# gwall-ceres/HighRes-net

Hardware: AMD Instinct MI355X
Metric: SR frames/sec (384x384 out) at B=32, n_views=32 (higher is better)
Workload: dtype bf16

## Files before the change

highres-net_amd/hrnet_hip/csrc/conv3x3.h:

```cpp
#pragma once
#include "common.h"

#define CONV_TILE_H 8
#define CONV_TILE_W 32
#define CONV_STEP_BYTES 8192

struct ConvParams {
    const void* in;
    const void* stack;
    int in_pair;
    void* out;
    const void* res;
    const float* alphas;
    const void* wpk;
    const float* bias;
    const float* slope;
    int M, H, W;
    int pair_h, pair_last, pair_vs;
    int out_h, out_vs;
    int res_mode;
    int alpha_vs, res_vs;
    int relu;
    const float* scale;
    size_t in_lo, stack_lo, out_lo, res_lo;
    const float* only_if_nonpos;
};

static inline size_t conv_packed_elems(int cin, int cout) { return (size_t)cin * cout * 9; }

int hrn_launch_conv3x3(int dt, int cin, int cout, const ConvParams& p, hipStream_t stream, bool general_only);

int hrn_launch_conv3x3_r64(const ConvParams& p, hipStream_t stream);

int hrn_launch_conv3x3_v6(int cin, int cout, const ConvParams& p, hipStream_t stream);

int hrn_launch_conv3x3_v6x3(int cin, int cout, const ConvParams& p, hipStream_t stream);

int hrn_launch_conv_pack(int dt, int cin, int cout, const float* w_oihw, void* packed, hipStream_t stream);
```

highres-net_amd/hrnet_hip/csrc/conv3x3_r64.hip:

```cpp
#include <type_traits>
#include "conv3x3.h"

namespace {

constexpr int HALO_H = CONV_TILE_H + 2;
constexpr int HALO_W = CONV_TILE_W + 2;
constexpr int IN_BYTES = HALO_H * HALO_W * 128;
constexpr int W_BYTES = 9 * 64 * 128;
constexpr int LDS_BYTES = W_BYTES + 2 * IN_BYTES + 256;

__device__ __forceinline__ void lds_done_then_barrier() {
    asm volatile("s_waitcnt lgkmcnt(0)" ::: "memory");
    __builtin_amdgcn_s_barrier();
    asm volatile("" ::: "memory");
}

__device__ __forceinline__ float raw_max(float a, float b) {
    float y;
    asm("v_max_f32 %0, %1, %2" : "=v"(y) : "v"(a), "v"(b));
    return y;
}

__device__ __attribute__((aligned(16))) unsigned hrn_r64_zero16[4];

template <bool RES>
__global__ __launch_bounds__(512, 2) void conv3x3_r64_kernel(const ConvParams p) {
    if (p.only_if_nonpos && p.only_if_nonpos[0] > 0.f) return;
    extern __shared__ __attribute__((aligned(16))) unsigned char smem[];
    unsigned char* w_lds = smem;
    float* bias_lds = (float*)(smem + W_BYTES + 2 * IN_BYTES);

    const int tid = threadIdx.x;
    const int lane = tid & 63;
    const int wave = __builtin_amdgcn_readfirstlane(tid >> 6);
    const int team = wave >> 2, tw = wave & 3;
    unsigned char* in_lds = smem + W_BYTES + team * IN_BYTES;
    const int r = lane & 31, hh = lane >> 5;
    const int H = p.H, W = p.W;
    const size_t hw = (size_t)H * W;
    const unsigned tiles_x = (W + CONV_TILE_W - 1) / CONV_TILE_W;
    const unsigned tiles_y = (H + CONV_TILE_H - 1) / CONV_TILE_H;
    const unsigned tiles = tiles_x * tiles_y;
    const unsigned total = tiles * (unsigned)p.M;
    const unsigned G = gridDim.x;
    const unsigned bid = blockIdx.x;
    const unsigned slot = (G & 7) == 0 ? (bid & 7) * (G >> 3) + (bid >> 3) : bid;
    if (slot >= total) return;
    const int ntl = (int)((total - slot + G - 1) / G);
    const int nmine = (ntl + 1 - team) >> 1;

    unsigned cur_m = (slot + team * G) / tiles, cur_t = (slot + team * G) - cur_m * tiles;
    const unsigned step_m = (2 * G) / tiles, step_t = 2 * G - step_m * tiles;

    {
        const u32x4* wg = (const u32x4*)p.wpk;
#pragma unroll
        for (int j = 0; j < W_BYTES / 16 / 512; ++j) {
            const int idx = tid + j * 512;
            const int row = idx >> 3, c = idx & 7;
            *(u32x4*)(w_lds + row * 128 + ((c ^ ((row >> 1) & 7)) << 4)) = wg[idx];
        }
        if (tid < 64) bias_lds[tid] = p.bias[tid];
    }

    unsigned voff[11], cm_lo = 0, cm_hi = 0;
    if (!RES) {
#pragma unroll
        for (int jj = 0; jj < 11; ++jj) {
            const int j = tw + 4 * jj;
            const int pix = j * 8 + (lane >> 3);
            const int py = pix / HALO_W, px = pix - py * HALO_W;
            voff[jj] = (unsigned)((py * W + px) * 128 + (((lane & 7) ^ ((pix >> 1) & 7)) << 4));
            unsigned cls = (py == 0 ? 1u : 0u) | (py == HALO_H - 1 ? 2u : 0u) | (px == 0 ? 4u : 0u) | (px == HALO_W - 1 ? 8u : 0u);
            if (pix >= HALO_H * HALO_W) cls = 0;
            if (jj < 8) cm_lo |= cls << (4 * jj); else cm_hi |= cls << (4 * (jj - 8));
        }
    }
    unsigned pend_F = 0;
    auto issue = [&](unsigned m, unsigned t) __attribute__((always_inline)) {
        const int ty = t / tiles_x;
        const int y0 = ty * CONV_TILE_H, x0 = (t - ty * tiles_x) * CONV_TILE_W;
        const unsigned char* base = (const unsigned char*)p.in + (size_t)m * hw * 128;
        const bool fast = !RES && y0 + CONV_TILE_H <= H && x0 + CONV_TILE_W <= W && (m > 0 || y0 > 0) &&
                          ((int)m + 1 < p.M || (size_t)(y0 + CONV_TILE_H) * W + x0 + CONV_TILE_W < hw);
        pend_F = 0;
        if (fast) {
            const unsigned char* hb = base + ((long)(y0 - 1) * W + (x0 - 1)) * 128;
#pragma unroll
            for (int jj = 0; jj < 11; ++jj) {
                const int j = tw + 4 * jj;
                if (j < 43) {
                    if (jj < 10 || j * 8 + (lane >> 3) < HALO_H * HALO_W)
                        __builtin_amdgcn_global_load_lds((const __attribute__((address_space(1))) void*)(hb + voff[jj]),
                                                         (__attribute__((address_space(3))) void*)(in_lds + j * 1024), 16, 0, 0);
                }
            }
            pend_F = (y0 == 0 ? 1u : 0u) | (y0 + CONV_TILE_H == H ? 2u : 0u) | (x0 == 0 ? 4u : 0u) | (x0 + CONV_TILE_W == W ? 8u : 0u);
            __builtin_amdgcn_sched_barrier(0);
            return;
        }
        int lq = lane;
        asm volatile("" : "+v"(lq));
#pragma unroll
        for (int jj = 0; jj < 11; ++jj) {
            const int j = tw + 4 * jj;
            if (j < 43) {
                const int pix = j * 8 + (lq >> 3);
                const int lc = (lq & 7) ^ ((pix >> 1) & 7);
                const int py = pix / HALO_W, px = pix - py * HALO_W;
                const int gy = y0 - 1 + py, gx = x0 - 1 + px;
                const bool ok = (unsigned)gy < (unsigned)H && (unsigned)gx < (unsigned)W;
                const unsigned char* src = ok ? base + (unsigned)((gy * W + gx) * 128 + lc * 16) : (const unsigned char*)hrn_r64_zero16;
                if (pix < HALO_H * HALO_W)
                    __builtin_amdgcn_global_load_lds((const __attribute__((address_space(1))) void*)src,
                                                     (__attribute__((address_space(3))) void*)(in_lds + j * 1024), 16, 0, 0);
            }
        }
        __builtin_amdgcn_sched_barrier(0);
    };
    auto fix_borders = [&]() __attribute__((always_inline)) {
        if (!RES && pend_F) {
            const unsigned fm = pend_F * 0x11111111u;
            const unsigned hit_lo = cm_lo & fm, hit_hi = cm_hi & fm;
            const u32x4 z = {0u, 0u, 0u, 0u};
#pragma unroll
            for (int jj = 0; jj < 11; ++jj) {
                const int j = tw + 4 * jj;
                if (j < 43) {
                    const unsigned h = jj < 8 ? (hit_lo >> (4 * jj)) & 15u : (hit_hi >> (4 * (jj - 8))) & 15u;
                    if (h) *(u32x4*)(in_lds + j * 1024 + lane * 16) = z;
                }
            }
        }
    };

    const bool has_slope = p.slope != nullptr;
    const float slope = has_slope ? p.slope[0] : 0.f;
    const bool slope01 = slope >= 0.f && slope <= 1.f;
    const unsigned lds0 = (unsigned)(__UINTPTR_TYPE__)(__attribute__((address_space(3))) unsigned char*)smem;
    unsigned a_off[4], a_off_hi[4], b_off[4][3];
#pragma unroll
    for (int ks = 0; ks < 4; ++ks) {
        a_off[ks] = lds0 + r * 128 + (((ks * 2 + hh) ^ ((r >> 1) & 7)) << 4);
        a_off_hi[ks] = a_off[ks] + 4 * 8192;
    }
#pragma unroll
    for (int row = 0; row < 4; ++row)
#pragma unroll
        for (int kx = 0; kx < 3; ++kx) {
            const int pix = (2 * tw + row) * HALO_W + r + kx;
            b_off[row][kx] = lds0 + (unsigned)(W_BYTES + team * IN_BYTES) + (((unsigned)pix << 7) | ((unsigned)(((pix >> 1) & 7) ^ hh) << 4));
        }

    f32x16 acc[2][2];

    auto multiply = [&]() __attribute__((always_inline)) {
#pragma unroll
        for (int cb = 0; cb < 2; ++cb)
#pragma unroll
            for (int g = 0; g < 4; ++g) {
                const f32x4 b = *(const f32x4*)(bias_lds + cb * 32 + 8 * g + 4 * hh);
#pragma unroll
                for (int j = 0; j < 4; ++j) { acc[cb][0][4 * g + j] = b[j]; acc[cb][1][4 * g + j] = b[j]; }
            }
        constexpr int NK = 36;
        bf16x8 fa[3][2], fb[3][2];
        auto rd = [&](bf16x8& dst, unsigned addr, int imm) __attribute__((always_inline)) {
            asm volatile("ds_read_b128 %0, %1 offset:%2" : "=v"(dst) : "v"(addr), "n"(imm));
        };
        auto load_part = [&](int i, int part) __attribute__((always_inline)) {
            const int s_ = i % 3, tap = i >> 2, ks = i & 3;
            const int ky = tap / 3, kx = tap - ky * 3;
            if (part < 2) {
                rd(fa[s_][part], tap < 4 ? a_off[ks] : a_off_hi[ks], (tap < 4 ? tap : tap - 4) * 8192 + part * 4096);
            } else {
                unsigned kbits = 0;
                if (ks) asm volatile("s_mov_b32 %0, %1" : "=s"(kbits) : "n"(ks << 5));
                rd(fb[s_][part - 2], b_off[part - 2 + ky][kx] ^ kbits, 0);
            }
        };
        asm volatile("s_waitcnt lgkmcnt(0)" ::: "memory");
        __builtin_amdgcn_s_setprio(3);
#pragma unroll
        for (int i = 0; i < 2; ++i)
#pragma unroll
            for (int part = 0; part < 4; ++part) load_part(i, part);
        __builtin_amdgcn_sched_barrier(0);
#pragma unroll
        for (int i = 0; i < NK; ++i) {
            const int s_ = i % 3;
            const bool more = i + 2 < NK;
            if (i < NK - 1) asm volatile("s_waitcnt lgkmcnt(5)" : "+v"(fa[s_][0]), "+v"(fb[s_][0]));
            else asm volatile("s_waitcnt lgkmcnt(1)" : "+v"(fa[s_][0]), "+v"(fb[s_][0]));
            acc[0][0] = __builtin_amdgcn_mfma_f32_32x32x16_bf16(fa[s_][0], fb[s_][0], acc[0][0], 0, 0, 0);
            if (more) load_part(i + 2, 0);
            __builtin_amdgcn_sched_barrier(0);
            if (more) asm volatile("s_waitcnt lgkmcnt(5)" : "+v"(fb[s_][1]));
            else if (i == NK - 2) asm volatile("s_waitcnt lgkmcnt(4)" : "+v"(fb[s_][1]));
            else asm volatile("s_waitcnt lgkmcnt(0)" : "+v"(fb[s_][1]));
            acc[0][1] = __builtin_amdgcn_mfma_f32_32x32x16_bf16(fa[s_][0], fb[s_][1], acc[0][1], 0, 0, 0);
            if (more) load_part(i + 2, 1);
            __builtin_amdgcn_sched_barrier(0);
            asm volatile("" : "+v"(fa[s_][1]));
            acc[1][0] = __builtin_amdgcn_mfma_f32_32x32x16_bf16(fa[s_][1], fb[s_][0], acc[1][0], 0, 0, 0);
            if (more) load_part(i + 2, 2);
            __builtin_amdgcn_sched_barrier(0);
            acc[1][1] = __builtin_amdgcn_mfma_f32_32x32x16_bf16(fa[s_][1], fb[s_][1], acc[1][1], 0, 0, 0);
            if (more) load_part(i + 2, 3);
            __builtin_amdgcn_sched_barrier(0);
        }
        __builtin_amdgcn_s_setprio(0);
    };

    u32x4 resv[2][4];
    float res_alpha = 1.f;
    auto fetch_residual = [&]() __attribute__((always_inline)) {
        const int m = (int)cur_m;
        const int ty = cur_t / tiles_x;
        const int y0 = ty * CONV_TILE_H, x0 = (cur_t - ty * tiles_x) * CONV_TILE_W;
        const unsigned char* rbase = (const unsigned char*)p.res + (size_t)m * hw * 128;
        if (p.res_mode == 3) {
            const int ob = m / p.out_h, oi = m - ob * p.out_h;
            rbase = (const unsigned char*)p.res + ((size_t)ob * p.res_vs + oi) * hw * 128;
            res_alpha = p.alphas ? p.alphas[(size_t)ob * p.alpha_vs + (p.pair_last - oi)] : 1.f;
        }
#pragma unroll
        for (int pb = 0; pb < 2; ++pb) {
            const int gy = y0 + 2 * tw + pb, gyc = gy < H ? gy : H - 1;
#pragma unroll
            for (int j = 0; j < 4; ++j) {
                const int gxj = x0 + (r & ~3) + j, gxjc = gxj < W ? gxj : W - 1;
                resv[pb][j] = __builtin_nontemporal_load((const u32x4*)(rbase + (unsigned)((gyc * W + gxjc) * 128 + hh * 64 + (r & 3) * 16)));
            }
        }
    };

    auto finish = [&](bool more) __attribute__((always_inline)) {
        const int m = (int)cur_m;
        const int ty = cur_t / tiles_x;
        const int y0 = ty * CONV_TILE_H, x0 = (cur_t - ty * tiles_x) * CONV_TILE_W;
        cur_t += step_t; cur_m += step_m;
        if (cur_t >= tiles) { cur_t -= tiles; ++cur_m; }
        size_t oimg = (size_t)m;
        int ob = 0, oi = 0;
        if (p.out_h > 0) { ob = m / p.out_h; oi = m - ob * p.out_h; oimg = (size_t)ob * p.out_vs + oi; }
        unsigned char* outp = (unsigned char*)p.out + (oimg * hw + (size_t)y0 * W + x0) * 128;
        if (RES) {
#pragma unroll
            for (int pb = 0; pb < 2; ++pb)
#pragma unroll
                for (int g = 0; g < 4; ++g) asm volatile("" :: "v"(resv[pb][g]));
            asm volatile("" :: "v"(res_alpha));
        }
        if (more) issue(cur_m, cur_t);
        auto epilogue = [&](auto act_c) __attribute__((always_inline)) {
        constexpr int ACT = decltype(act_c)::value;
#pragma unroll
        for (int pb = 0; pb < 2; ++pb) {
            const int gy = y0 + 2 * tw + pb;
            u32x4 uu[4];
            if (RES) quad_transpose(resv[pb], (lane & 1) != 0, (lane & 2) != 0);
#pragma unroll
            for (int g = 0; g < 4; ++g) {
                float xa[4], xb[4];
#pragma unroll
                for (int j = 0; j < 4; ++j) { xa[j] = acc[0][pb][4 * g + j]; xb[j] = acc[1][pb][4 * g + j]; }
                if (ACT == 1) {
#pragma unroll
                    for (int j = 0; j < 4; ++j) { xa[j] = raw_max(xa[j], slope * xa[j]); xb[j] = raw_max(xb[j], slope * xb[j]); }
                } else if (ACT == 2) {
#pragma unroll
                    for (int j = 0; j < 4; ++j) { xa[j] = xa[j] >= 0.f ? xa[j] : slope * xa[j]; xb[j] = xb[j] >= 0.f ? xb[j] : slope * xb[j]; }
                }
                u32x4 u;
                if (RES) {
                    float v[8];
#pragma unroll
                    for (int j = 0; j < 4; ++j) {
                        const u32x2 sw = __builtin_amdgcn_permlane32_swap(__float_as_uint(xa[j]), __float_as_uint(xb[j]), false, false);
                        v[j] = __uint_as_float(sw[0]);
                        v[4 + j] = __uint_as_float(sw[1]);
                    }
                    const u32x4 rq = resv[pb][g];
#pragma unroll
                    for (int j = 0; j < 4; ++j) {
                        const float r0 = __uint_as_float(rq[j] << 16), r1 = __uint_as_float(rq[j] & 0xffff0000u);
                        if (p.res_mode == 3) { v[2 * j] = r0 + res_alpha * v[2 * j]; v[2 * j + 1] = r1 + res_alpha * v[2 * j + 1]; }
                        else { v[2 * j] += r0; v[2 * j + 1] += r1; }
                    }
#pragma unroll
                    for (int j = 0; j < 4; ++j) u[j] = pack2_bf16(v[2 * j], v[2 * j + 1]);
                } else {
                    const u32x2 s0 = __builtin_amdgcn_permlane32_swap(pack2_bf16(xa[0], xa[1]), pack2_bf16(xb[0], xb[1]), false, false);
                    const u32x2 s1 = __builtin_amdgcn_permlane32_swap(pack2_bf16(xa[2], xa[3]), pack2_bf16(xb[2], xb[3]), false, false);
                    u[0] = s0[0]; u[1] = s1[0]; u[2] = s0[1]; u[3] = s1[1];
                }
                uu[g] = u;
            }
            {
                quad_transpose(uu, (lane & 1) != 0, (lane & 2) != 0);
                unsigned char* oq = outp + (unsigned)(((2 * tw + pb) * W + (r & ~3)) * 128 + hh * 64 + (r & 3) * 16);
#pragma unroll
                for (int j = 0; j < 4; ++j)
                    if (gy < H && x0 + (r & ~3) + j < W) __builtin_nontemporal_store(uu[j], (u32x4*)(oq + j * 128));
            }
        }
        };
        if (!has_slope) epilogue(std::integral_constant<int, 0>{});
        else if (slope01) epilogue(std::integral_constant<int, 1>{});
        else epilogue(std::integral_constant<int, 2>{});
        {
            const int nst = 4 * ((y0 + 2 * tw < H) + (y0 + 2 * tw + 1 < H));
            if (nst == 8) asm volatile("s_waitcnt vmcnt(8)" ::: "memory");
            else if (nst == 4) asm volatile("s_waitcnt vmcnt(4)" ::: "memory");
            else asm volatile("s_waitcnt vmcnt(0)" ::: "memory");
        }
        fix_borders();
    };

    if (nmine > 0) issue(cur_m, cur_t);
    asm volatile("s_waitcnt vmcnt(0)" ::: "memory");
    fix_borders();
    lds_done_then_barrier();

    for (int ph = 0; ph <= ntl; ++ph) {
        const int q = ph - team;
        if (q >= 0) {
            const int k = q >> 1;
            if (k < nmine) {
                if ((q & 1) == 0) { if (RES) fetch_residual(); multiply(); }
                else finish(k + 1 < nmine);
            }
        }
        if (ph < ntl) lds_done_then_barrier();
    }
}


template <bool RES>
int launch_r64(const ConvParams& p, long grid, hipStream_t stream) {
    { const int rc_lds = hrn_allow_lds((const void*)conv3x3_r64_kernel<RES>, LDS_BYTES); if (rc_lds) return rc_lds; }
    hipLaunchKernelGGL(conv3x3_r64_kernel<RES>, dim3((unsigned)grid), dim3(512), LDS_BYTES, stream, p);
    HRN_LAUNCH_CHECK();
    return 0;
}

}

int hrn_launch_conv3x3_r64(const ConvParams& p, hipStream_t stream) {
    if (p.scale || p.relu || p.in_pair || p.res_mode == 2) return -100;
    static_assert(LDS_BYTES <= 160 * 1024, "LDS budget");
    const long tiles = (long)((p.W + CONV_TILE_W - 1) / CONV_TILE_W) * ((p.H + CONV_TILE_H - 1) / CONV_TILE_H);
    const long total = tiles * p.M;
    HRN_CHECK(total > 0, -2, "conv3x3_r64: bad tile count %ld", total);
    if (total >= (1L << 30) || (long)p.H * p.W * 128 >= (1L << 31)) return -100;
    long grid = hrn_device_cus();
    if (total < grid) grid = total;
    if (grid >= 8) grid &= ~7L;
    const double px = (double)p.M * p.H * p.W;
    HrnProfScope prof(p.res_mode ? "conv3x3_bf16_64x64+res" : "conv3x3_bf16_64x64", 2.0 * 64 * 64 * 9 * px,
                      px * 2 * (64 + 64 + (p.res_mode ? 64 : 0)), stream);
    return p.res_mode ? launch_r64<true>(p, grid, stream) : launch_r64<false>(p, grid, stream);
}
```

Measured before the change: 1969.

## Walk conv tiles in vertical strips with a ring buffer reusing halo rows

The 64x64 3x3 conv kernel now assigns each team a vertical segment of consecutive tiles in one column, rather than scattered tiles. The input LDS tile becomes a ring buffer, so the two halo rows shared with the previous tile are kept and only the new rows are loaded. This cuts redundant global loads of halo rows by roughly 20 percent of input traffic. A host heuristic picks the segment length to balance the load across CUs. The cost is more complex indexing, per-tile recomputation of the B-operand offsets, and possible load imbalance or tail effects.

```diff
diff --git a/highres-net_amd/hrnet_hip/csrc/conv3x3.h b/highres-net_amd/hrnet_hip/csrc/conv3x3.h
--- a/highres-net_amd/hrnet_hip/csrc/conv3x3.h
+++ b/highres-net_amd/hrnet_hip/csrc/conv3x3.h
@@ -23,6 +23,8 @@
     int relu;
     const float* scale;
     size_t in_lo, stack_lo, out_lo, res_lo;
+    int r64_walk;
+    int r64_seg;
     const float* only_if_nonpos;
 };
 
diff --git a/highres-net_amd/hrnet_hip/csrc/conv3x3_r64.hip b/highres-net_amd/hrnet_hip/csrc/conv3x3_r64.hip
--- a/highres-net_amd/hrnet_hip/csrc/conv3x3_r64.hip
+++ b/highres-net_amd/hrnet_hip/csrc/conv3x3_r64.hip
@@ -5,9 +5,15 @@
 
 constexpr int HALO_H = CONV_TILE_H + 2;
 constexpr int HALO_W = CONV_TILE_W + 2;
-constexpr int IN_BYTES = HALO_H * HALO_W * 128;
+constexpr int HALO_PIX = HALO_H * HALO_W;
+constexpr int TOP_PIECES = 9;
+constexpr int NEW_PIECES = 34;
+constexpr int RING_PIECES = TOP_PIECES + NEW_PIECES;
+constexpr int RING_PIX = RING_PIECES * 8;
+constexpr int RING_BYTES = RING_PIECES * 1024;
 constexpr int W_BYTES = 9 * 64 * 128;
-constexpr int LDS_BYTES = W_BYTES + 2 * IN_BYTES + 256;
+constexpr int LDS_BYTES = W_BYTES + 2 * RING_BYTES + 256;
+static_assert(HALO_PIX + 4 == RING_PIX && 2 * HALO_W + 4 == TOP_PIECES * 8 && CONV_TILE_H * HALO_W == NEW_PIECES * 8, "ring geometry");
 
 __device__ __forceinline__ void lds_done_then_barrier() {
     asm volatile("s_waitcnt lgkmcnt(0)" ::: "memory");
@@ -28,29 +34,68 @@
     if (p.only_if_nonpos && p.only_if_nonpos[0] > 0.f) return;
     extern __shared__ __attribute__((aligned(16))) unsigned char smem[];
     unsigned char* w_lds = smem;
-    float* bias_lds = (float*)(smem + W_BYTES + 2 * IN_BYTES);
+    float* bias_lds = (float*)(smem + W_BYTES + 2 * RING_BYTES);
 
     const int tid = threadIdx.x;
     const int lane = tid & 63;
     const int wave = __builtin_amdgcn_readfirstlane(tid >> 6);
     const int team = wave >> 2, tw = wave & 3;
-    unsigned char* in_lds = smem + W_BYTES + team * IN_BYTES;
+    unsigned char* in_lds = smem + W_BYTES + team * RING_BYTES;
     const int r = lane & 31, hh = lane >> 5;
     const int H = p.H, W = p.W;
     const size_t hw = (size_t)H * W;
     const unsigned tiles_x = (W + CONV_TILE_W - 1) / CONV_TILE_W;
     const unsigned tiles_y = (H + CONV_TILE_H - 1) / CONV_TILE_H;
-    const unsigned tiles = tiles_x * tiles_y;
-    const unsigned total = tiles * (unsigned)p.M;
+    const unsigned L = (unsigned)p.r64_seg;
+    const unsigned segs = (tiles_y + L - 1) / L;
+    const unsigned short_by = segs * L - tiles_y;
+    const unsigned items = tiles_x * segs * (unsigned)p.M;
     const unsigned G = gridDim.x;
     const unsigned bid = blockIdx.x;
     const unsigned slot = (G & 7) == 0 ? (bid & 7) * (G >> 3) + (bid >> 3) : bid;
-    if (slot >= total) return;
-    const int ntl = (int)((total - slot + G - 1) / G);
-    const int nmine = (ntl + 1 - team) >> 1;
-
-    unsigned cur_m = (slot + team * G) / tiles, cur_t = (slot + team * G) - cur_m * tiles;
-    const unsigned step_m = (2 * G) / tiles, step_t = 2 * G - step_m * tiles;
+    if (slot >= items) return;
+    auto team_tiles = [&](unsigned tt) -> int {
+        const unsigned first = slot + tt * G;
+        if (first >= items) return 0;
+        unsigned n = ((items - first + 2 * G - 1) / (2 * G)) * L;
+        if (short_by)
+            for (unsigned it = first; it < items; it += 2 * G)
+                if ((it / tiles_x) % segs == segs - 1) n -= short_by;
+        return (int)n;
+    };
+    const int n0 = team_tiles(0), n1 = team_tiles(1);
+    const int nmine = team ? n1 : n0;
+    const int nph = 2 * n0 > 2 * n1 + 1 ? 2 * n0 : 2 * n1 + 1;
+
+    unsigned c_m, c_tx, c_sg, c_i = 0, sp = 0;
+    {
+        const unsigned row = (slot + team * G) / tiles_x;
+        c_tx = (slot + team * G) - row * tiles_x;
+        c_m = row / segs;
+        c_sg = row - c_m * segs;
+    }
+    const unsigned step_row = (2 * G) / tiles_x, step_tx = 2 * G - step_row * tiles_x;
+    const unsigned step_m = step_row / segs, step_sg = step_row - step_m * segs;
+    unsigned c_len = c_sg + 1 == segs ? L - short_by : L;
+    auto advance = [&]() __attribute__((always_inline)) -> bool {
+        if (c_i + 1 < c_len) {
+            ++c_i;
+            sp += NEW_PIECES;
+            if (sp >= (unsigned)RING_PIECES) sp -= RING_PIECES;
+            return true;
+        }
+        unsigned carry = 0;
+        c_tx += step_tx;
+        if (c_tx >= tiles_x) { c_tx -= tiles_x; carry = 1; }
+        c_sg += step_sg + carry;
+        carry = 0;
+        if (c_sg >= segs) { c_sg -= segs; carry = 1; }
+        c_m += step_m + carry;
+        c_i = 0;
+        sp = 0;
+        c_len = c_sg + 1 == segs ? L - short_by : L;
+        return false;
+    };
 
     {
         const u32x4* wg = (const u32x4*)p.wpk;
@@ -63,72 +108,94 @@
         if (tid < 64) bias_lds[tid] = p.bias[tid];
     }
 
-    unsigned voff[11], cm_lo = 0, cm_hi = 0;
+    unsigned voff[9], cm = 0;
     if (!RES) {
 #pragma unroll
-        for (int jj = 0; jj < 11; ++jj) {
-            const int j = tw + 4 * jj;
-            const int pix = j * 8 + (lane >> 3);
+        for (int jj = 0; jj < 9; ++jj) {
+            const int k = tw + 4 * jj;
+            const int pix = 2 * HALO_W + k * 8 + (lane >> 3);
             const int py = pix / HALO_W, px = pix - py * HALO_W;
-            voff[jj] = (unsigned)((py * W + px) * 128 + (((lane & 7) ^ ((pix >> 1) & 7)) << 4));
-            unsigned cls = (py == 0 ? 1u : 0u) | (py == HALO_H - 1 ? 2u : 0u) | (px == 0 ? 4u : 0u) | (px == HALO_W - 1 ? 8u : 0u);
-            if (pix >= HALO_H * HALO_W) cls = 0;
-            if (jj < 8) cm_lo |= cls << (4 * jj); else cm_hi |= cls << (4 * (jj - 8));
+            voff[jj] = (unsigned)((py * W + px) * 128 + (((lane & 7) ^ (lane >> 4)) << 4));
+            unsigned cls = (py == HALO_H - 1 ? 1u : 0u) | (px == 0 ? 2u : 0u) | (px == HALO_W - 1 ? 4u : 0u);
+            if (k >= NEW_PIECES) cls = 0;
+            cm |= cls << (3 * jj);
         }
     }
     unsigned pend_F = 0;
-    auto issue = [&](unsigned m, unsigned t) __attribute__((always_inline)) {
-        const int ty = t / tiles_x;
-        const int y0 = ty * CONV_TILE_H, x0 = (t - ty * tiles_x) * CONV_TILE_W;
+    auto ring_piece = [&](int k) __attribute__((always_inline)) -> unsigned {
+        unsigned pc = sp + TOP_PIECES + k;
+        if (pc >= (unsigned)RING_PIECES) pc -= RING_PIECES;
+        return pc;
+    };
+    auto issue = [&](bool first) __attribute__((always_inline)) {
+        const unsigned m = c_m;
+        const int y0 = (int)(c_sg * L + c_i) * CONV_TILE_H, x0 = (int)c_tx * CONV_TILE_W;
         const unsigned char* base = (const unsigned char*)p.in + (size_t)m * hw * 128;
+        if (first) {
+            int lq = lane;
+            asm volatile("" : "+v"(lq));
+#pragma unroll
+            for (int jj = 0; jj < 3; ++jj) {
+                const int j = tw + 4 * jj;
+                if (j < TOP_PIECES) {
+                    const int rp = j * 8 + (lq >> 3), pix = rp - 4;
+                    const int lc = (lq & 7) ^ ((rp >> 1) & 7);
+                    const int py = pix >= HALO_W ? 1 : 0, px = pix - py * HALO_W;
+                    const int gy = y0 - 1 + py, gx = x0 - 1 + px;
+                    const bool ok = pix >= 0 && (unsigned)gy < (unsigned)H && (unsigned)gx < (unsigned)W;
+                    const unsigned char* src = ok ? base + (unsigned)((gy * W + gx) * 128 + lc * 16) : (const unsigned char*)hrn_r64_zero16;
+                    if (pix >= 0)
+                        __builtin_amdgcn_global_load_lds((const __attribute__((address_space(1))) void*)src,
+                                                         (__attribute__((address_space(3))) void*)(in_lds + j * 1024), 16, 0, 0);
+                }
+            }
+        }
         const bool fast = !RES && y0 + CONV_TILE_H <= H && x0 + CONV_TILE_W <= W && (m > 0 || y0 > 0) &&
                           ((int)m + 1 < p.M || (size_t)(y0 + CONV_TILE_H) * W + x0 + CONV_TILE_W < hw);
         pend_F = 0;
         if (fast) {
             const unsigned char* hb = base + ((long)(y0 - 1) * W + (x0 - 1)) * 128;
 #pragma unroll
-            for (int jj = 0; jj < 11; ++jj) {
-                const int j = tw + 4 * jj;
-                if (j < 43) {
-                    if (jj < 10 || j * 8 + (lane >> 3) < HALO_H * HALO_W)
-                        __builtin_amdgcn_global_load_lds((const __attribute__((address_space(1))) void*)(hb + voff[jj]),
-                                                         (__attribute__((address_space(3))) void*)(in_lds + j * 1024), 16, 0, 0);
+            for (int jj = 0; jj < 9; ++jj) {
+                const int k = tw + 4 * jj;
+                if (k < NEW_PIECES) {
+                    const unsigned pc = ring_piece(k);
+                    __builtin_amdgcn_global_load_lds((const __attribute__((address_space(1))) void*)(hb + (voff[jj] ^ ((pc & 1) << 6))),
+                                                     (__attribute__((address_space(3))) void*)(in_lds + pc * 1024), 16, 0, 0);
                 }
             }
-            pend_F = (y0 == 0 ? 1u : 0u) | (y0 + CONV_TILE_H == H ? 2u : 0u) | (x0 == 0 ? 4u : 0u) | (x0 + CONV_TILE_W == W ? 8u : 0u);
+            pend_F = (y0 + CONV_TILE_H == H ? 1u : 0u) | (x0 == 0 ? 2u : 0u) | (x0 + CONV_TILE_W == W ? 4u : 0u);
             __builtin_amdgcn_sched_barrier(0);
             return;
         }
         int lq = lane;
         asm volatile("" : "+v"(lq));
 #pragma unroll
-        for (int jj = 0; jj < 11; ++jj) {
-            const int j = tw + 4 * jj;
-            if (j < 43) {
-                const int pix = j * 8 + (lq >> 3);
-                const int lc = (lq & 7) ^ ((pix >> 1) & 7);
+        for (int jj = 0; jj < 9; ++jj) {
+            const int k = tw + 4 * jj;
+            if (k < NEW_PIECES) {
+                const unsigned pc = ring_piece(k);
+                const int pix = 2 * HALO_W + k * 8 + (lq >> 3);
+                const int lc = (lq & 7) ^ (lq >> 4) ^ (int)((pc & 1) << 2);
                 const int py = pix / HALO_W, px = pix - py * HALO_W;
                 const int gy = y0 - 1 + py, gx = x0 - 1 + px;
                 const bool ok = (unsigned)gy < (unsigned)H && (unsigned)gx < (unsigned)W;
                 const unsigned char* src = ok ? base + (unsigned)((gy * W + gx) * 128 + lc * 16) : (const unsigned char*)hrn_r64_zero16;
-                if (pix < HALO_H * HALO_W)
-                    __builtin_amdgcn_global_load_lds((const __attribute__((address_space(1))) void*)src,
-                                                     (__attribute__((address_space(3))) void*)(in_lds + j * 1024), 16, 0, 0);
+                __builtin_amdgcn_global_load_lds((const __attribute__((address_space(1))) void*)src,
+                                                 (__attribute__((address_space(3))) void*)(in_lds + pc * 1024), 16, 0, 0);
             }
         }
         __builtin_amdgcn_sched_barrier(0);
     };
     auto fix_borders = [&]() __attribute__((always_inline)) {
         if (!RES && pend_F) {
-            const unsigned fm = pend_F * 0x11111111u;
-            const unsigned hit_lo = cm_lo & fm, hit_hi = cm_hi & fm;
+            const unsigned hit = cm & (pend_F * 0x1249249u);
             const u32x4 z = {0u, 0u, 0u, 0u};
 #pragma unroll
-            for (int jj = 0; jj < 11; ++jj) {
-                const int j = tw + 4 * jj;
-                if (j < 43) {
-                    const unsigned h = jj < 8 ? (hit_lo >> (4 * jj)) & 15u : (hit_hi >> (4 * (jj - 8))) & 15u;
-                    if (h) *(u32x4*)(in_lds + j * 1024 + lane * 16) = z;
+            for (int jj = 0; jj < 9; ++jj) {
+                const int k = tw + 4 * jj;
+                if (k < NEW_PIECES) {
+                    if ((hit >> (3 * jj)) & 7u) *(u32x4*)(in_lds + ring_piece(k) * 1024 + lane * 16) = z;
                 }
             }
         }
@@ -144,13 +211,18 @@
         a_off[ks] = lds0 + r * 128 + (((ks * 2 + hh) ^ ((r >> 1) & 7)) << 4);
         a_off_hi[ks] = a_off[ks] + 4 * 8192;
     }
-#pragma unroll
-    for (int row = 0; row < 4; ++row)
-#pragma unroll
-        for (int kx = 0; kx < 3; ++kx) {
-            const int pix = (2 * tw + row) * HALO_W + r + kx;
-            b_off[row][kx] = lds0 + (unsigned)(W_BYTES + team * IN_BYTES) + (((unsigned)pix << 7) | ((unsigned)(((pix >> 1) & 7) ^ hh) << 4));
-        }
+    auto set_b_off = [&]() __attribute__((always_inline)) {
+        const unsigned first = sp * 8 + 4 + 2 * tw * HALO_W + r;
+#pragma unroll
+        for (int row = 0; row < 4; ++row)
+#pragma unroll
+            for (int kx = 0; kx < 3; ++kx) {
+                unsigned pix = first + row * HALO_W + kx;
+                if (pix >= (unsigned)RING_PIX) pix -= RING_PIX;
+                b_off[row][kx] = lds0 + (unsigned)(W_BYTES + team * RING_BYTES) + ((pix << 7) | ((((pix >> 1) & 7) ^ hh) << 4));
+            }
+    };
+    set_b_off();
 
     f32x16 acc[2][2];
 
@@ -215,9 +287,8 @@
     u32x4 resv[2][4];
     float res_alpha = 1.f;
     auto fetch_residual = [&]() __attribute__((always_inline)) {
-        const int m = (int)cur_m;
-        const int ty = cur_t / tiles_x;
-        const int y0 = ty * CONV_TILE_H, x0 = (cur_t - ty * tiles_x) * CONV_TILE_W;
+        const int m = (int)c_m;
+        const int y0 = (int)(c_sg * L + c_i) * CONV_TILE_H, x0 = (int)c_tx * CONV_TILE_W;
         const unsigned char* rbase = (const unsigned char*)p.res + (size_t)m * hw * 128;
         if (p.res_mode == 3) {
             const int ob = m / p.out_h, oi = m - ob * p.out_h;
@@ -236,11 +307,9 @@
     };
 
     auto finish = [&](bool more) __attribute__((always_inline)) {
-        const int m = (int)cur_m;
-        const int ty = cur_t / tiles_x;
-        const int y0 = ty * CONV_TILE_H, x0 = (cur_t - ty * tiles_x) * CONV_TILE_W;
-        cur_t += step_t; cur_m += step_m;
-        if (cur_t >= tiles) { cur_t -= tiles; ++cur_m; }
+        const int m = (int)c_m;
+        const int y0 = (int)(c_sg * L + c_i) * CONV_TILE_H, x0 = (int)c_tx * CONV_TILE_W;
+        const bool turn = advance();
         size_t oimg = (size_t)m;
         int ob = 0, oi = 0;
         if (p.out_h > 0) { ob = m / p.out_h; oi = m - ob * p.out_h; oimg = (size_t)ob * p.out_vs + oi; }
@@ -252,7 +321,7 @@
                 for (int g = 0; g < 4; ++g) asm volatile("" :: "v"(resv[pb][g]));
             asm volatile("" :: "v"(res_alpha));
         }
-        if (more) issue(cur_m, cur_t);
+        if (more) { issue(!turn); set_b_off(); }
         auto epilogue = [&](auto act_c) __attribute__((always_inline)) {
         constexpr int ACT = decltype(act_c)::value;
 #pragma unroll
@@ -318,12 +387,12 @@
         fix_borders();
     };
 
-    if (nmine > 0) issue(cur_m, cur_t);
+    if (nmine > 0) issue(true);
     asm volatile("s_waitcnt vmcnt(0)" ::: "memory");
     fix_borders();
     lds_done_then_barrier();
 
-    for (int ph = 0; ph <= ntl; ++ph) {
+    for (int ph = 0; ph < nph; ++ph) {
         const int q = ph - team;
         if (q >= 0) {
             const int k = q >> 1;
@@ -332,7 +401,7 @@
                 else finish(k + 1 < nmine);
             }
         }
-        if (ph < ntl) lds_done_then_barrier();
+        if (ph + 1 < nph) lds_done_then_barrier();
     }
 }
 
@@ -345,20 +414,36 @@
     return 0;
 }
 
+int r64_segment(long strips, long tiles_y, long teams) {
+    long best = 1, best_cost = -1;
+    for (long L = 1; L <= tiles_y && L <= 64; ++L) {
+        const long items = strips * ((tiles_y + L - 1) / L);
+        const long cost = ((items + teams - 1) / teams) * L;
+        if (best_cost < 0 || cost <= best_cost) { best = L; best_cost = cost; }
+    }
+    return (int)best;
+}
+
 }
 
 int hrn_launch_conv3x3_r64(const ConvParams& p, hipStream_t stream) {
     if (p.scale || p.relu || p.in_pair || p.res_mode == 2) return -100;
     static_assert(LDS_BYTES <= 160 * 1024, "LDS budget");
-    const long tiles = (long)((p.W + CONV_TILE_W - 1) / CONV_TILE_W) * ((p.H + CONV_TILE_H - 1) / CONV_TILE_H);
-    const long total = tiles * p.M;
+    const long tiles_x = (p.W + CONV_TILE_W - 1) / CONV_TILE_W, tiles_y = (p.H + CONV_TILE_H - 1) / CONV_TILE_H;
+    const long total = tiles_x * tiles_y * p.M;
     HRN_CHECK(total > 0, -2, "conv3x3_r64: bad tile count %ld", total);
     if (total >= (1L << 30) || (long)p.H * p.W * 128 >= (1L << 31)) return -100;
-    long grid = hrn_device_cus();
-    if (total < grid) grid = total;
+    static const int env_walk = [] { const char* e = getenv("HRN_R64_WALK"); return e ? atoi(e) : 0; }();
+    const int walk = p.r64_walk ? p.r64_walk : env_walk;
+    const long cus = hrn_device_cus();
+    ConvParams q = p;
+    q.r64_seg = walk == 1 ? 1 : walk == 2 ? (int)tiles_y : r64_segment(tiles_x * p.M, tiles_y, 2 * cus);
+    const long items = tiles_x * p.M * ((tiles_y + q.r64_seg - 1) / q.r64_seg);
+    long grid = cus;
+    if (items < grid) grid = items;
     if (grid >= 8) grid &= ~7L;
     const double px = (double)p.M * p.H * p.W;
     HrnProfScope prof(p.res_mode ? "conv3x3_bf16_64x64+res" : "conv3x3_bf16_64x64", 2.0 * 64 * 64 * 9 * px,
                       px * 2 * (64 + 64 + (p.res_mode ? 64 : 0)), stream);
-    return p.res_mode ? launch_r64<true>(p, grid, stream) : launch_r64<false>(p, grid, stream);
-}
+    return p.res_mode ? launch_r64<true>(q, grid, stream) : launch_r64<false>(q, grid, stream);
+}
```

Result: no change. 1965 (-0.2%).
